# nilsfriess/dune-ddm

Hardware: AMD Instinct MI355X
Metric: preconditioned CG iterations/sec (two-level additive Schwarz), 3D Poisson 10M DoF (higher is better)
Workload: dtype f64

## Files before the change

### dune-ddm_amd/__init__.py

```python
from __future__ import annotations

import ctypes
import os

import numpy as np

_HERE = os.path.dirname(os.path.abspath(__file__))
LIB_PATH = os.path.join(_HERE, "libddm_hip.so")

GENEO_AVAILABLE = True

DDM_OK, DDM_EINVAL, DDM_EHIP, DDM_ENOTIMPL, DDM_ENUMERIC, DDM_ECOMM = 0, -1, -2, -3, -4, -5


class DdmError(RuntimeError):
    def __init__(self, code, msg):
        super().__init__(f"ddm_hip error {code}: {msg}")
        self.code = code


class SolveResult(ctypes.Structure):
    _fields_ = [("iterations", ctypes.c_int32), ("converged", ctypes.c_int32), ("def0", ctypes.c_double),
                ("reduction", ctypes.c_double), ("elapsed_s", ctypes.c_double)]

# ... 104 lines not shown
    "ddm_geneo_params_default": (_I32, [ctypes.POINTER(GeneoParams)]),
    "ddm_geneo_basis": (_I32, [_P, _P, _P, _I64, _P, _P, _P, ctypes.POINTER(GeneoParams), _I64, _P, _P, _P, ctypes.POINTER(GeneoInfo)]),
    "ddm_msgfem_basis": (_I32, [_P, _P, _P, _I64, _P, _P, _P, _P, ctypes.POINTER(GeneoParams), _I64, _P, _P, _P, ctypes.POINTER(GeneoInfo)]),
    "ddm_svd_basis": (_I32, [_P, _P, _I64, _P, _P, _P, _P, _I32, _I32, _D, _I32, _P, _P, ctypes.POINTER(GeneoInfo)]),
    "ddm_harmonic_create": (_I32, [_P, _P, _I64, _P, _I64, _P, _I64, _P, _PP]),
    "ddm_harmonic_destroy": (None, [_P]),
    "ddm_harmonic_extend": (_I32, [_P, _P, _I32, _P, _I64]),
    "ddm_blockvec_gram": (_I32, [_P, _I64, _P, _P, _I64, _I32, _P, _I64, _I32, _P]),
    "ddm_blockvec_gram2_sym": (_I32, [_P, _I64, _P, _P, _I64, _P, _P, _I64, _I32, _P, _P]),
    "ddm_blockvec_rotate": (_I32, [_P, _I64, _P, _P, _I64, _I32, _P, _I32, _P, _I64, _P, _I64]),
    "ddm_dense_sym_eig_host": (_I32, [_I32, _P, _P]),
    "ddm_dense_rayleigh_ritz_host": (_I32, [_I32, _P, _P, _I32, _D, _P, _P]),
    "ddm_combined_create": (_I32, [_P, _I32, _P, _P, _P, _PP]),
    "ddm_combined_destroy": (None, [_P]),
    "ddm_combined_apply": (_I32, [_P, _P, _P, _P]),
    "ddm_cg_solve": (_I32, [_P, _P, _P, _P, _P, _D, _I32, _I32, _P, ctypes.POINTER(SolveResult)]),
    "ddm_gmres_solve": (_I32, [_P, _P, _P, _P, _P, _D, _I32, _I32, _P, ctypes.POINTER(SolveResult)]),
    "ddm_bicgstab_solve": (_I32, [_P, _P, _P, _P, _P, _D, _I32, _P, ctypes.POINTER(ctypes.c_int32), ctypes.POINTER(SolveResult)]),
    "ddm_op_apply_multi": (_I32, [_P, _P, _I32, _P, _P]),
    "ddm_op_applyscaleadd_multi": (_I32, [_P, _P, _I32, _D, _P, _P]),
    "ddm_dot_multi": (_I32, [_P, _P, _I32, _P, _P, _P]),
    "ddm_schwarz_apply_multi": (_I32, [_P, _P, _I32, _P, _P]),
    "ddm_galerkin_apply_multi": (_I32, [_P, _P, _I32, _P, _P]),
    "ddm_combined_apply_multi": (_I32, [_P, _P, _I32, _P, _P]),
    "ddm_cg_solve_multi": (_I32, [_P, _P, _P, _I32, _P, _P, _D, _I32, _P, ctypes.POINTER(SolveResult)]),
    "ddm_cg_solve_queue": (_I32, [_P, _P, _P, _I64, _I32, _P, _P, _D, _I32, _P, ctypes.POINTER(SolveResult)]),
    "ddm_bicgstab_solve_queue": (_I32, [_P, _P, _P, _I64, _I32, _P, _P, _D, _I32, _P, ctypes.POINTER(ctypes.c_int32), ctypes.POINTER(SolveResult)]),
    "ddm_gmres_solve_multi": (_I32, [_P, _P, _P, _I32, _P, _P, _D, _I32, _I32, _P, ctypes.POINTER(SolveResult)]),
    "ddm_fgmres_solve": (_I32, [_P, _P, _P, _P, _P, _D, _I32, _I32, _P, ctypes.POINTER(SolveResult)]),
    "ddm_fgmres_solve_multi": (_I32, [_P, _P, _P, _I32, _P, _P, _D, _I32, _I32, _P, ctypes.POINTER(SolveResult)]),
# ... 474 lines not shown
    MODES = {"additive": 0, "multiplicative": 1}

    def __init__(self, ctx: Context, mode="additive", op=None, schwarz=None, galerkin=None):
        if mode not in self.MODES:
            raise NotImplementedError("Unknown apply mode in CombinedPreconditioner, use either additive or multiplicative")
        self.ctx = ctx
        h = ctypes.c_void_p()
        ctx.check(ctx.lib.ddm_combined_create(ctx.h, self.MODES[mode], op.h if op else None, schwarz.h if schwarz else None,
                                              galerkin.h if galerkin else None, ctypes.byref(h)))
        self.h = h
        self._keep = (op, schwarz, galerkin)

    def apply(self, x, d):
        self.ctx.check(self.ctx.lib.ddm_combined_apply(self.ctx.h, self.h, _ptr(x), _ptr(d)))

    def apply_multi(self, X, D):
        self.ctx.check(self.ctx.lib.ddm_combined_apply_multi(self.ctx.h, self.h, _ncols(X, D), _ptr(X), _ptr(D)))

    def check_status(self):
        self.ctx.check(self.ctx.lib.ddm_combined_status(self.ctx.h, self.h))


def cg_solve(ctx: Context, op: NonOverlappingOperator, prec: CombinedPreconditioner, x, b, reduction=1e-10, maxit=1000,
             fixed_iterations=0, history=True):
    res = SolveResult()
    hist = np.zeros(max(maxit, fixed_iterations) + 1, dtype=np.float64) if history else None
    ctx.check(ctx.lib.ddm_cg_solve(ctx.h, op.h, prec.h, _ptr(x), _ptr(b), float(reduction), int(maxit), int(fixed_iterations),
                                   _hp(hist), ctypes.byref(res)))
    return res, (hist[:res.iterations + 1] if history else None)

# ... 297 lines not shown
def dia_windows_host(A):
    lib = load_library()
    n = A.shape[0]
    rp, ci, va = _np(A.indptr, np.int64), _np(A.indices, np.int32), _np(A.data, np.float64)
    max_segs, max_runs = n + 1, 32 * (n + 1)
    segs = np.zeros((max_segs, 4), dtype=np.int32)
    runs = np.zeros((max_runs, 3), dtype=np.int32)
    counts = np.zeros(4, dtype=np.int64)
    rc = lib.ddm_dia_windows_host(n, _hp(rp), _hp(ci), _hp(va), max_segs, _hp(segs), max_runs, _hp(runs), _hp(counts))
    if rc != DDM_OK:
        raise ValueError("ddm_dia_windows_host: bad arguments")
    out = [dict(staged=bool(s[0]), window=int(s[2]), runs=[tuple(r) for r in runs[s[3]:s[3] + s[1]].tolist()]) for s in segs[:counts[0]]]
    return out, int(counts[2])


def blockvec_gram(ctx: Context, sub_ptr, U, V):
    bp = _np(sub_ptr, np.int64)
    assert U.is_contiguous() and V.is_contiguous() and U.shape[0] == V.shape[0] == bp[-1]
    out = np.empty((len(bp) - 1, U.shape[1], V.shape[1]), dtype=np.float64)
    ctx.check(ctx.lib.ddm_blockvec_gram(ctx.h, len(bp) - 1, _hp(bp), _ptr(U), U.stride(0), U.shape[1], _ptr(V), V.stride(0), V.shape[1], _hp(out)))
    return out


def blockvec_gram2_sym(ctx: Context, sub_ptr, U, V1, V2):
    bp = _np(sub_ptr, np.int64)
    p = U.shape[1]
    assert V1.shape == U.shape == V2.shape and V1.stride(0) == V2.stride(0) and U.shape[0] == bp[-1]
    g1 = np.empty((len(bp) - 1, p, p), dtype=np.float64)
    g2 = np.empty_like(g1)
    ctx.check(ctx.lib.ddm_blockvec_gram2_sym(ctx.h, len(bp) - 1, _hp(bp), _ptr(U), U.stride(0), _ptr(V1), _ptr(V2), V1.stride(0), p, _hp(g1), _hp(g2)))
# ... 9 lines not shown
```

### dune-ddm_amd/csrc/ddm_hip.hip

```cpp
#include "../../include/ddm_hip.h"

#include <dlfcn.h>
#include <rccl/rccl.h>

#include <algorithm>
#include <atomic>
#include <chrono>
#include <cmath>
#include <cstdarg>
#include <cstdio>
#include <cstdlib>
#include <cstring>
#include <deque>
#include <map>
#include <memory>
#include <mutex>
#include <string>
#include <thread>
#include <type_traits>
#include <vector>

#include "host_vec.hpp"
#include "device_buffer.hpp"
#include "kernels.hpp"
// ... 8 lines not shown

using namespace ddm;

#include "context.hpp"
#include "csr.hpp"
#include "local_factor.hpp"
#include "tri_levels.hpp"
#include "tri_csr.hpp"
#include "engine_xcd2.hpp"
#include "engine_pipe.hpp"
#include "engine_box.hpp"
#include "local_solve.hpp"
#include "local_solver.hpp"
#include "geneo.hpp"
#include "halo.hpp"
#include "preconditioners.hpp"
#include "krylov.hpp"

extern "C" int ddm_dense_sym_eig_host(int n, double *V, double *w) { return dense::sym_eig(n, V, w) ? DDM_OK : DDM_ENUMERIC; }
extern "C" int ddm_dense_rayleigh_ritz_host(int p, const double *gA, const double *gC, int keep, double tau, double *mu, double *Y)
{
  return dense::rayleigh_ritz(p, gA, gC, keep, tau, mu, Y);
}
extern "C" int ddm_dense_sym_pinv_host(int m, const double *W, double tol, double *Wpinv, int *rank)
{
  if (m < 1 || !W || !Wpinv || !rank || W == Wpinv || !(tol > 0.0 && tol < 1.0)) return fail(nullptr, DDM_EINVAL, "ddm_dense_sym_pinv_host: bad arguments");
  return dense::sym_pinv(m, W, tol, Wpinv, rank) ? DDM_OK : DDM_ENUMERIC;
}
extern "C" int ddm_dense_bgmres_factor_host(int p, const double *G, const double *scale2, double tol, double *S, double *C, int *rank)
{
// ... 22 lines not shown
```

### dune-ddm_amd/csrc/halo.hpp

```cpp
#pragma once

struct ddm_halo {
  int tag = 0, mode = 0;
  int64_t nsend = 0, nrecv = 0, ndst = 0, self_off_send = 0, self_off_recv = 0, self_count = 0;
  dbuf<int64_t> send_idx, dst_idx, dst_ptr, src_pos;
  dbuf<double> sendbuf, recvbuf;
  bool remote = false;
  std::vector<int64_t> send_counts, recv_counts;
  dbuf<double> msend, mrecv;
  int mcols = 0;
};

extern "C" int ddm_halo_create(ddm_ctx *ctx, int tag, int mode, int64_t nsend, const int64_t *send_idx,
                               const int64_t *send_counts, const int64_t *recv_counts, int64_t ndst, const int64_t *dst_idx,
                               const int64_t *dst_ptr, const int64_t *src_pos, ddm_halo **out)
{
  if (!ctx || !out || (mode != 0 && mode != 1)) return fail(ctx, DDM_EINVAL, "ddm_halo_create: bad arguments");
  auto H = std::make_unique<ddm_halo>();
  H->tag = tag;
  H->mode = mode;
  H->nsend = nsend;
  H->ndst = ndst;
  H->send_counts.assign(send_counts, send_counts + ctx->nranks);
  H->recv_counts.assign(recv_counts, recv_counts + ctx->nranks);
// ... 2 lines not shown
    if (r == ctx->rank) {
      H->self_off_send = ssum;
      H->self_off_recv = rsum;
      H->self_count = send_counts[r];
      if (send_counts[r] != recv_counts[r]) return fail(ctx, DDM_EINVAL, "halo: self send/recv counts differ");
    } else if (send_counts[r] || recv_counts[r])
      H->remote = true;
    ssum += send_counts[r];
    rsum += recv_counts[r];
  }
  if (ssum != nsend) return fail(ctx, DDM_EINVAL, "halo: send_counts do not sum to nsend");
  H->nrecv = rsum;
  const int64_t nsrc = ndst > 0 ? dst_ptr[ndst] : 0;
  for (int64_t k = 0; k < nsrc; ++k)
    if (src_pos[k] < 0 || src_pos[k] >= rsum) return fail(ctx, DDM_EINVAL, "halo: src_pos out of range");
  int rc = upload(ctx, send_idx, nsend, H->send_idx);
  if (!rc) rc = upload(ctx, dst_idx, ndst, H->dst_idx);
  if (!rc) rc = upload(ctx, dst_ptr, ndst + 1, H->dst_ptr);
  if (!rc) rc = upload(ctx, src_pos, nsrc, H->src_pos);
  if (!rc && H->sendbuf.alloc(nsend) != hipSuccess) rc = DDM_EHIP;
  if (!rc && H->recvbuf.alloc(rsum) != hipSuccess) rc = DDM_EHIP;
  if (rc) return fail(ctx, rc, "halo: device allocation failed");
  *out = H.release();
  return DDM_OK;
}
extern "C" void ddm_halo_destroy(ddm_halo *H) { delete H; }
extern "C" double *ddm_halo_sendbuf(ddm_halo *H) { return H->sendbuf; }
extern "C" double *ddm_halo_recvbuf(ddm_halo *H) { return H->recvbuf; }

static int halo_wire_rccl(ddm_ctx *ctx, const ddm_halo *H, int64_t m, const double *send, double *recv)
// ... 81 lines not shown
```

### dune-ddm_amd/csrc/kernels.hpp

```cpp
#pragma once
#include <hip/hip_runtime.h>
#include <stdint.h>

namespace ddm {

constexpr int WG = 256;
constexpr int SPMV_NNZ = 2048;
constexpr int RED_MAX_BLOCKS = 1024;
constexpr int RED_TRIPS = 4;

__device__ __forceinline__ int xcd_remap(int orig, int nwg)
{
  const int q = nwg >> 3, r = nwg & 7, xcd = orig & 7;
  return (xcd < r ? xcd * (q + 1) : r * (q + 1) + (xcd - r) * q) + (orig >> 3);
}

__device__ __forceinline__ double wave_sum(double v)
{
#pragma unroll
  for (int o = 32; o > 0; o >>= 1) v += __shfl_down(v, o, 64);
  return v;
}

__device__ __forceinline__ double block_sum(double v, double *lds4)
// ... 1074 lines not shown
      if (own[u]) s += a[u] * b[u];
  }
  for (; i < n; i += step)
    if (!MASKED || mask[i]) s += x[i] * y[i];
  s = block_sum(s, red);
  if (threadIdx.x == 0) partial[blockIdx.x] = s;
}
__global__ __launch_bounds__(WG) void k_reduce_final(int nb, const double *__restrict__ partial, double *__restrict__ out)
{
  __shared__ double red[4];
  double s = 0.0;
  for (int i = threadIdx.x; i < nb; i += WG) s += partial[i];
  s = block_sum(s, red);
  if (threadIdx.x == 0) out[0] = s;
}

__global__ void k_cg_lambda(double *scal) { scal[2] = scal[0] / scal[1]; }
__global__ void k_cg_beta(double *scal)
{
  scal[4] = scal[3] / scal[0];
  scal[0] = scal[3];
}
__global__ void k_cg_update(int64_t n, const double *__restrict__ scal, const double *__restrict__ p,
                            const double *__restrict__ q, double *__restrict__ x, double *__restrict__ b)
{
  const double lam = scal[2];
  for (int64_t i = blockIdx.x * (int64_t)WG + threadIdx.x; i < n; i += (int64_t)gridDim.x * WG) {
    x[i] += lam * p[i];
    b[i] -= lam * q[i];
  }
// ... 321 lines not shown
```

### dune-ddm_amd/csrc/krylov.hpp

```cpp
#pragma once

struct StreamDrain {
  ddm_ctx *ctx;
  ~StreamDrain() { (void)hipStreamSynchronize(ctx->stream); }
};

static void solve_result_reset(ddm_solve_result *res) { *res = ddm_solve_result{0, 0, 0.0, 1.0, 0.0}; }
enum class Defect0 { NaN, Zero, Go };
static Defect0 classify_initial_defect(double def0) { return !(def0 == def0) ? Defect0::NaN : def0 < 1e-30 ? Defect0::Zero : Defect0::Go; }
static int krylov_finish(ddm_ctx *ctx, const ddm_combined *prec, int rc, std::chrono::steady_clock::time_point t0, double *elapsed_s)
{
  (void)hipStreamSynchronize(ctx->stream);
  *elapsed_s = std::chrono::duration<double>(std::chrono::steady_clock::now() - t0).count();
  if (rc || !prec->schwarz) return rc;
  int st = 0;
  rc = ddm_ilu0_status(ctx, prec->schwarz->solver, &st);
  if (!rc && st) rc = fail(ctx, DDM_ENUMERIC, "persistent triangular solve timed out waiting for a level (results invalid)");
  return rc;
}

struct MultiFrame {
  ddm_ctx *ctx;
  const char *what;
  int m;
// ... 82 lines not shown
extern "C" void ddm_cg_end(ddm_ctx *ctx, ddm_cg *S)
{
  if (ctx) ctx->piggy = nullptr;
  if (!S) return;
  if (ctx) (void)hipStreamSynchronize(ctx->stream);
  delete S;
}
extern "C" double ddm_cg_def0(const ddm_cg *S) { return S->def0; }
extern "C" int ddm_cg_steps(ddm_ctx *ctx, ddm_cg *S, int k)
{
  struct PiggyGuard { ddm_ctx *ctx; ~PiggyGuard() { ctx->piggy = nullptr; } } piggy_guard{ctx};
  double *scal = ctx->scal;
  const int G = grid_for(S->n);
  for (int i = 0; i < k; ++i) {
    const bool first = S->it == 0;
    DDMCHECK(ddm_combined_apply(ctx, S->prec, first ? S->p : S->q, S->b));
    DDMCHECK(dot_device(ctx, S->n, S->op->owner, first ? S->p : S->q, S->b, scal + (first ? 0 : 3)));
    if (!first) {
      hipLaunchKernelGGL(k_cg_beta, dim3(1), dim3(1), 0, ctx->stream, scal);
      hipLaunchKernelGGL(k_cg_direction, dim3(G), dim3(WG), 0, ctx->stream, S->n, scal, S->q, S->p);
    }
    DDMCHECK(ddm_op_apply(ctx, S->op, S->p, S->q));
    DDMCHECK(dot_device(ctx, S->n, S->op->owner, S->p, S->q, scal + 1));
    hipLaunchKernelGGL(k_cg_lambda, dim3(1), dim3(1), 0, ctx->stream, scal);
    {
      const int nb = grid_for(S->n, WG * 4, RED_MAX_BLOCKS);
      if (S->op->owner)
        hipLaunchKernelGGL(k_cg_update_norm<true>, dim3(nb), dim3(WG), 0, ctx->stream, S->n, scal, S->op->owner, S->p, S->q, S->x, S->b, ctx->partial);
      else
        hipLaunchKernelGGL(k_cg_update_norm<false>, dim3(nb), dim3(WG), 0, ctx->stream, S->n, scal, S->op->owner, S->p, S->q, S->x, S->b, ctx->partial);
      hipLaunchKernelGGL(k_reduce_final, dim3(1), dim3(WG), 0, ctx->stream, nb, ctx->partial, scal + 5);
      if (i + 1 < k && S->prec->galerkin) ctx->piggy = scal + 5;
// ... 1559 lines not shown
```

### dune-ddm_amd/csrc/preconditioners.hpp

```cpp
#pragma once

static int dot_device(ddm_ctx *ctx, int64_t n, const uint8_t *mask, const double *x, const double *y, double *result_dev)
{
  const int nb = grid_for(n, WG * 4, RED_MAX_BLOCKS);
  if (mask)
    hipLaunchKernelGGL(k_dot_partial<true>, dim3(nb), dim3(WG), 0, ctx->stream, n, mask, x, y, ctx->partial);
  else
    hipLaunchKernelGGL(k_dot_partial<false>, dim3(nb), dim3(WG), 0, ctx->stream, n, mask, x, y, ctx->partial);
  hipLaunchKernelGGL(k_reduce_final, dim3(1), dim3(WG), 0, ctx->stream, nb, ctx->partial, result_dev);
  HIPCHECK(ctx, hipGetLastError());
  DDMCHECK(ctx_allreduce(ctx, result_dev, 1, "scalar product"));
  return DDM_OK;
}

template <class Launch>
static void for_column_groups(int m, Launch &&launch)
{
  for (int c0 = 0; c0 < m;) {
    const int cb = m - c0 >= 8 ? 8 : m - c0 >= 4 ? 4 : m - c0 >= 2 ? 2 : 1;
    launch(c0, cb);
    c0 += cb;
  }
}
#define DDM_MULTI_CB_DISPATCH(KERNEL, MASKED, cb, ...)                                                                 \
  do {                                                                                                                 \
    if (MASKED) {                                                                                                      \
      if (cb == 8) hipLaunchKernelGGL((KERNEL<8, true>), __VA_ARGS__);                                                 \
// ... 136 lines not shown
  DDMCHECK(dot_multi_device(ctx, op->n, op->owner, nrhs, X, Y, out));
  return ddm_memcpy_d2h(ctx, result_host, out, sizeof(double) * (size_t)nrhs);
}

struct ddm_schwarz {
  int64_t n = 0, n_novlp = 0;
  int type = 1;
  ddm_ilu0 *solver = nullptr;
  dbuf<int32_t> ext_map;
  dbuf<double> pou;
  dbuf<double> d_ovlp, x_ovlp;
  ddm_halo *copy = nullptr, *add = nullptr;
  dbuf<double> md_ovlp, mx_ovlp;
  int mcols = 0;
  bool multi_f32 = false;
  ~ddm_schwarz() { ddm_ilu0_destroy(solver); }
};
extern "C" int ddm_schwarz_create(ddm_ctx *ctx, const ddm_csr *A_dir, int64_t nblocks, const int64_t *block_ptr, int64_t n_novlp,
                                  const int32_t *ext_map_host, const double *pou_host, int type, ddm_halo *ovlp_copy,
                                  ddm_halo *ovlp_add, ddm_schwarz **out)
{
  return ddm_schwarz_create_ex(ctx, A_dir, nblocks, block_ptr, n_novlp, ext_map_host, pou_host, type, "ilu0", ovlp_copy, ovlp_add, out);
}
extern "C" int ddm_schwarz_create_ex(ddm_ctx *ctx, const ddm_csr *A_dir, int64_t nblocks, const int64_t *block_ptr, int64_t n_novlp,
                                     const int32_t *ext_map_host, const double *pou_host, int type, const char *subdomain_solver,
                                     ddm_halo *ovlp_copy, ddm_halo *ovlp_add, ddm_schwarz **out)
{
  if (!ctx || !A_dir || !out || !ext_map_host) return fail(ctx, DDM_EINVAL, "ddm_schwarz_create: bad arguments");
  const std::string st = subdomain_solver ? subdomain_solver : "ilu0";
  const bool direct = st == "cholmod" || st == "direct" || st == "cholesky" || st == "umfpack" || st == "ldl";
// ... 38 lines not shown
extern "C" int ddm_schwarz_engine(const ddm_schwarz *S) { return S ? ddm_ilu0_engine(S->solver) : -1; }
extern "C" ddm_ilu0 *ddm_schwarz_local_solver(ddm_schwarz *S) { return S ? S->solver : nullptr; }
extern "C" int ddm_schwarz_status(ddm_ctx *ctx, const ddm_schwarz *S)
{
  if (!S) return fail(ctx, DDM_EINVAL, "ddm_schwarz_status: bad arguments");
  int st = 0;
  DDMCHECK(ddm_ilu0_status(ctx, S->solver, &st));
  if (st) return fail(ctx, DDM_ENUMERIC, "local triangular solve timed out waiting for a dependency (code %d): results are invalid", st);
  return DDM_OK;
}
static int local_status_check(ddm_ctx *ctx, const ddm_schwarz *S)
{
  if (const unsigned e = S ? ilu0_peek_status(S->solver) : 0u)
    return fail(ctx, DDM_ENUMERIC, "an earlier local triangular solve timed out waiting for a dependency (code %u): results since then are invalid", e);
  return DDM_OK;
}
static int schwarz_apply_impl(ddm_ctx *ctx, ddm_schwarz *S, double *x, const double *d, bool acc)
{
  DDMCHECK(local_status_check(ctx, S));
  {
    ScopedTimer t(ctx, "Schwarz/get defect");
    hipLaunchKernelGGL(k_extend, dim3(grid_for(S->n)), dim3(WG), 0, ctx->stream, S->n, S->ext_map, d, S->d_ovlp);
    DDMCHECK(ddm_halo_exchange(ctx, S->copy, S->d_ovlp));
  }
  {
    ScopedTimer t(ctx, "Schwarz/local solve");
    DDMCHECK(ddm_ilu0_solve(ctx, S->solver, S->d_ovlp, S->x_ovlp));
  }
  {
    ScopedTimer t(ctx, "Schwarz/add solution");
// ... 255 lines not shown
      hipLaunchKernelGGL(k_coarse_restrict_partial, dim3(nchunk), dim3(WG), 0, ctx->stream, (int)nleft, n, left, y, chunks, partial, nchunk);
    hipLaunchKernelGGL(k_coarse_restrict_final, dim3(1), dim3(WG), 0, ctx->stream, 1, (int)nleft, d_scp, partial, d_cidx, nleft, outd + j * nleft);
  }
  if (!rc) rc = ddm_memcpy_d2h(ctx, out_host, outd, sizeof(double) * (size_t)(nleft * nright));
  return rc;
}

constexpr bool OVERLAP_DEFAULT = true;
constexpr int OVERLAP_WAVES_PER_16_CU = 7, OVERLAP_KMAX_MEASURED = 20;
static int overlap_default_grid(int num_cu, int64_t kmax)
{
  const int64_t k = std::max<int64_t>(kmax, OVERLAP_KMAX_MEASURED);
  const int64_t g = (OVERLAP_WAVES_PER_16_CU * num_cu * k + 16 * OVERLAP_KMAX_MEASURED - 1) / (16 * OVERLAP_KMAX_MEASURED);
  return (int)std::max<int64_t>(1, std::min<int64_t>(g, num_cu));
}
struct ddm_combined {
  int mode = 0;
  ddm_op *op = nullptr;
  ddm_schwarz *schwarz = nullptr;
  ddm_galerkin *galerkin = nullptr;
  dbuf<double> dnext;
  int64_t n = 0;
  bool fused = false;
  int overlap = 0;
  int side_grid = 0;
  dbuf<double> mdnext, mp, mq;
  dbuf<double> mxw, mbw;
  dbuf<int64_t> mqueue_tab;
  dbuf<double> mrt, mv, my;
  dbuf<double> mz;
  int mcols = 0, mcg_cols = 0, mqueue_cols = 0, mbicg_cols = 0, mbcg_cols = 0;
};
extern "C" int ddm_combined_create(ddm_ctx *ctx, int mode, ddm_op *op, ddm_schwarz *schwarz, ddm_galerkin *galerkin, ddm_combined **out)
{
  if (!ctx || !out || !schwarz) return fail(ctx, DDM_EINVAL, "ERROR: No preconditioners added yet");
  if (mode != 0 && mode != 1) return fail(ctx, DDM_ENOTIMPL, "Unknown apply mode in CombinedPreconditioner, use either additive or multiplicative");
  if (mode == 1 && galerkin && !op) return fail(ctx, DDM_EINVAL, "ERROR: ApplyMode is multiplicative but operator A is not provided. Set with `set_op`");
  auto C = std::make_unique<ddm_combined>();
  C->mode = mode;
  C->op = op;
  C->schwarz = schwarz;
  C->galerkin = galerkin;
  C->n = schwarz->n_novlp;
  if (mode == 0 && galerkin) {
    const char *f = std::getenv("DDM_FUSE_LEVELS");
    const char *e = std::getenv("DDM_OVERLAP_COARSE");
    const char *g = std::getenv("DDM_OVERLAP_GRID");
    C->fused = !(f && f[0] == '0') && galerkin->copy == schwarz->copy && galerkin->add == schwarz->add && galerkin->n == schwarz->n && galerkin->n_novlp == schwarz->n_novlp;
    if (C->fused && (ctx->nranks == 1 || ctx->rccl)) C->overlap = e ? (e[0] == '1' ? 1 : 0) : (OVERLAP_DEFAULT ? 2 : 0);
    C->side_grid = g ? std::max(1, std::atoi(g)) : overlap_default_grid(ctx->num_cu, galerkin->kmax);
  }
  if (C->dnext.alloc(C->n) != hipSuccess) return fail(ctx, DDM_EHIP, "combined: allocation failed");
  *out = C.release();
  return DDM_OK;
}
extern "C" int ddm_combined_status(ddm_ctx *ctx, const ddm_combined *C)
{
  if (!C) return fail(ctx, DDM_EINVAL, "ddm_combined_status: bad arguments");
  return C->schwarz ? ddm_schwarz_status(ctx, C->schwarz) : DDM_OK;
}
extern "C" void ddm_combined_destroy(ddm_combined *C) { delete C; }
static int combined_apply_fused(ddm_ctx *ctx, ddm_combined *C, double *x, const double *d)
{
  ddm_schwarz *S = C->schwarz;
  ddm_galerkin *G = C->galerkin;
  bool pipe_engine = false;
  if (C->overlap != 0) DDMCHECK(ilu0_is_pipe(ctx, S->solver, &pipe_engine));
  const bool two_streams = C->overlap == 1 || (C->overlap == 2 && pipe_engine);
  if (two_streams) DDMCHECK(ctx_side_stream(ctx));
  {
    ScopedTimer t(ctx, "Schwarz/get defect");
    hipLaunchKernelGGL(k_extend, dim3(grid_for(S->n)), dim3(WG), 0, ctx->stream, S->n, S->ext_map, d, S->d_ovlp);
    DDMCHECK(ddm_halo_exchange(ctx, S->copy, S->d_ovlp));
  }
  auto timed_chain = [&](int spread_grid) -> int {
    ScopedTimer t(ctx, "GalerkinPrec/apply");
    return coarse_chain(ctx, G, S->d_ovlp, spread_grid);
  };
  if (two_streams) {
    HIPCHECK(ctx, hipEventRecord(ctx->ev_fork, ctx->stream));
    hipStream_t main = ctx->stream;
    HIPCHECK(ctx, hipStreamWaitEvent(ctx->side, ctx->ev_fork, 0));
    ctx->stream = ctx->side;
    const int rc = timed_chain(C->side_grid);
    const hipError_t e = hipEventRecord(ctx->ev_join, ctx->side);
    ctx->stream = main;
    if (rc) return rc;
    if (e != hipSuccess) return fail(ctx, DDM_EHIP, "hipEventRecord failed: %s", hipGetErrorString(e));
// ... 1 lines not shown
  const double *pou = S->type == 1 ? S->pou : nullptr;
  if (!two_streams) DDMCHECK(timed_chain(0));
  const bool fold = !two_streams || pipe_engine;
  {
    ScopedTimer t(ctx, "Schwarz/local solve");
    DDMCHECK(ilu0_solve_epilogue(ctx, S->solver, S->d_ovlp, S->x_ovlp, fold ? pou : nullptr, fold ? (const double *)G->x_ovlp : nullptr,
                                 two_streams && fold ? ctx->ev_join : nullptr));
  }
  {
    ScopedTimer t(ctx, "Schwarz/add solution");
    if (!fold) {
      if (pou) hipLaunchKernelGGL(k_scale, dim3(grid_for(S->n)), dim3(WG), 0, ctx->stream, S->n, pou, S->x_ovlp);
      HIPCHECK(ctx, hipStreamWaitEvent(ctx->stream, ctx->ev_join, 0));
      hipLaunchKernelGGL(k_axpy, dim3(grid_for(S->n)), dim3(WG), 0, ctx->stream, S->n, 1.0, (const double *)G->x_ovlp, S->x_ovlp);
    }
    DDMCHECK(ddm_halo_exchange(ctx, S->add, S->x_ovlp));
    hipLaunchKernelGGL((k_restrict<false, false>), dim3(grid_for(S->n)), dim3(WG), 0, ctx->stream, S->n, S->ext_map, S->x_ovlp, (const double *)nullptr, x);
    HIPCHECK(ctx, hipGetLastError());
  }
  return DDM_OK;
}

extern "C" int ddm_combined_apply(ddm_ctx *ctx, ddm_combined *C, double *x, const double *d)
{
  ScopedTimer t(ctx, "CombinedPreconditioner/apply");
  DDMCHECK(local_status_check(ctx, C->schwarz));
  if (C->mode == 0 && C->galerkin && C->fused) return combined_apply_fused(ctx, C, x, d);
  DDMCHECK(schwarz_apply_impl(ctx, C->schwarz, x, d, false));
  if (!C->galerkin) return DDM_OK;
  if (C->mode == 0) {
    static const bool no_share = std::getenv("DDM_NO_SHARED_DEFECT") != nullptr;
    const bool share = !no_share && C->galerkin->copy == C->schwarz->copy && C->galerkin->n == C->schwarz->n && C->galerkin->n_novlp == C->schwarz->n_novlp;
    return galerkin_apply_impl(ctx, C->galerkin, x, d, true, share ? C->schwarz->d_ovlp : nullptr);
  }
  HIPCHECK(ctx, hipMemcpyAsync(C->dnext, d, sizeof(double) * (size_t)C->n, hipMemcpyDeviceToDevice, ctx->stream));
  DDMCHECK(ddm_op_applyscaleadd(ctx, C->op, -1.0, x, C->dnext));
  return galerkin_apply_impl(ctx, C->galerkin, x, C->dnext, true);
}
static int combined_apply_multi_impl(ddm_ctx *ctx, ddm_combined *C, int m, double *X, const double *D)
{
  ScopedTimer t(ctx, "CombinedPreconditioner/apply");
  ddm_schwarz *S = C->schwarz;
  ddm_galerkin *G = C->galerkin;
  DDMCHECK(local_status_check(ctx, S));
  if (C->mode == 0 && G && C->fused) {
    DDMCHECK(schwarz_multi_scratch(ctx, S, m));
    DDMCHECK(galerkin_multi_scratch(ctx, G, m));
    {
      ScopedTimer t2(ctx, "Schwarz/get defect");
      hipLaunchKernelGGL(k_extend_multi, dim3(grid_for(S->n * m)), dim3(WG), 0, ctx->stream, S->n, m, S->ext_map, D, S->md_ovlp);
      DDMCHECK(halo_exchange_multi(ctx, S->copy, m, S->md_ovlp));
    }
// ... 33 lines not shown
```

### include/ddm_hip.h

```cpp
#ifndef DDM_HIP_H
#define DDM_HIP_H

#include <stdint.h>

#ifdef __cplusplus
extern "C" {
#endif

#define DDM_OK 0
#define DDM_EINVAL (-1)
#define DDM_EHIP (-2)
#define DDM_ENOTIMPL (-3)
#define DDM_ENUMERIC (-4)
#define DDM_ECOMM (-5)

typedef struct ddm_ctx ddm_ctx;
typedef struct ddm_csr ddm_csr;
typedef struct ddm_ilu0 ddm_ilu0;
typedef struct ddm_halo ddm_halo;
typedef struct ddm_op ddm_op;
typedef struct ddm_schwarz ddm_schwarz;
typedef struct ddm_galerkin ddm_galerkin;
typedef struct ddm_combined ddm_combined;

// ... 150 lines not shown
int ddm_harmonic_extend(ddm_ctx *ctx, ddm_harmonic *H, int nrhs, double *X, int64_t ldx);
int ddm_blockvec_gram(ddm_ctx *ctx, int64_t nsub, const int64_t *sub_ptr, const double *U, int64_t ldu, int pu, const double *V, int64_t ldv,
                      int pv, double *G_host);
int ddm_blockvec_gram2_sym(ddm_ctx *ctx, int64_t nsub, const int64_t *sub_ptr, const double *U, int64_t ldu, const double *V1, const double *V2, int64_t ldv, int p,
                           double *G1_host, double *G2_host);
int ddm_blockvec_rotate(ddm_ctx *ctx, int64_t nsub, const int64_t *sub_ptr, const double *U, int64_t ldu, int p, const double *Y_host, int q,
                        const double *Base, int64_t ldb, double *Out, int64_t ldo);
int ddm_dense_sym_eig_host(int n, double *V, double *w);
int ddm_dense_rayleigh_ritz_host(int p, const double *gA, const double *gC, int keep, double tau, double *mu, double *Y);

int ddm_combined_create(ddm_ctx *ctx, int mode, ddm_op *op, ddm_schwarz *schwarz, ddm_galerkin *galerkin,
                        ddm_combined **out);
void ddm_combined_destroy(ddm_combined *C);
int ddm_combined_status(ddm_ctx *ctx, const ddm_combined *C);
int ddm_combined_apply(ddm_ctx *ctx, ddm_combined *C, double *x, const double *d);

typedef struct {
  int32_t iterations;
  int32_t converged;
  double def0;
  double reduction;
  double elapsed_s;
} ddm_solve_result;
int ddm_cg_solve(ddm_ctx *ctx, ddm_op *op, ddm_combined *prec, double *x, double *b, double reduction, int maxit,
                 int fixed_iterations, double *hist_host, ddm_solve_result *res);

int ddm_gmres_solve(ddm_ctx *ctx, ddm_op *op, ddm_combined *prec, double *x, double *b, double reduction, int maxit,
                    int restart, double *hist_host, ddm_solve_result *res);

int ddm_fgmres_solve(ddm_ctx *ctx, ddm_op *op, ddm_combined *prec, double *x, double *b, double reduction, int maxit, int restart,
// ... 70 lines not shown
```

Measured before the change: 228.3.

## Precompute rank-local halo plans and fuse restriction with preconditioned dot

On a single rank the copy and add halo exchanges are turned into precomputed gather plans. The extend kernel reads directly from the right source index, so the copy exchange pass disappears. The add exchange becomes a small sum kernel over shared rows, followed by a restriction that takes owned values or the sums. That restriction also accumulates the CG dot product, which removes a separate dot kernel and extra vector reads each iteration. In exchange it adds plan-building and host-copy setup, more code paths, and depends on the halo being rank-local.

```diff
diff --git a/dune-ddm_amd/__init__.py b/dune-ddm_amd/__init__.py
--- a/dune-ddm_amd/__init__.py
+++ b/dune-ddm_amd/__init__.py
@@ -142,6 +142,9 @@
     "ddm_combined_create": (_I32, [_P, _I32, _P, _P, _P, _PP]),
     "ddm_combined_destroy": (None, [_P]),
     "ddm_combined_apply": (_I32, [_P, _P, _P, _P]),
+    "ddm_combined_apply_dot": (_I32, [_P, _P, _P, _P, ctypes.POINTER(ctypes.c_double)]),
+    "ddm_combined_local_passes": (_I32, [_P]),
+    "ddm_local_passes_host": (_I32, [_I64, _I64, _P, _I64, _I64, _P, _I64, _I64, _P, _P, _P, _P, _P, _P]),
     "ddm_cg_solve": (_I32, [_P, _P, _P, _P, _P, _D, _I32, _I32, _P, ctypes.POINTER(SolveResult)]),
     "ddm_gmres_solve": (_I32, [_P, _P, _P, _P, _P, _D, _I32, _I32, _P, ctypes.POINTER(SolveResult)]),
     "ddm_bicgstab_solve": (_I32, [_P, _P, _P, _P, _P, _D, _I32, _P, ctypes.POINTER(ctypes.c_int32), ctypes.POINTER(SolveResult)]),
@@ -646,6 +649,14 @@
     def apply(self, x, d):
         self.ctx.check(self.ctx.lib.ddm_combined_apply(self.ctx.h, self.h, _ptr(x), _ptr(d)))
 
+    def apply_dot(self, x, d):
+        r = ctypes.c_double()
+        self.ctx.check(self.ctx.lib.ddm_combined_apply_dot(self.ctx.h, self.h, _ptr(x), _ptr(d), ctypes.byref(r)))
+        return r.value
+
+    def local_passes(self):
+        return int(self.ctx.lib.ddm_combined_local_passes(self.h))
+
     def apply_multi(self, X, D):
         self.ctx.check(self.ctx.lib.ddm_combined_apply_multi(self.ctx.h, self.h, _ncols(X, D), _ptr(X), _ptr(D)))
 
@@ -973,6 +984,25 @@
     return out, int(counts[2])
 
 
+def local_passes_host(n_novlp, ext_map, copy_plan, add_plan, d, x_ovlp):
+    lib = load_library()
+    em = _np(ext_map, np.int32)
+    n = len(em)
+    d, xo = _np(d, np.float64), _np(x_ovlp, np.float64)
+    assert len(d) == n_novlp and len(xo) == n
+    args, keep = [], []
+    for plan in (copy_plan, add_plan):
+        a = [_np(plan[k], np.int64) for k in ("send_idx", "dst_idx", "dst_ptr", "src_pos")]
+        keep.append(a)
+        args += [len(a[0]), len(a[1]), (ctypes.c_void_p * 4)(*[x.ctypes.data for x in a])]
+    d_ovlp, z = np.full(n, np.nan), np.full(n_novlp, np.nan)
+    counts = np.zeros(3, dtype=np.int64)
+    rc = lib.ddm_local_passes_host(n, int(n_novlp), _hp(em), *args, _hp(d), _hp(d_ovlp), _hp(xo), _hp(z), _hp(counts))
+    if rc != DDM_OK:
+        raise ValueError("ddm_local_passes_host: bad arguments")
+    return (d_ovlp, z, dict(sums=int(counts[1]), sources=int(counts[2]))) if counts[0] else None
+
+
 def blockvec_gram(ctx: Context, sub_ptr, U, V):
     bp = _np(sub_ptr, np.int64)
     assert U.is_contiguous() and V.is_contiguous() and U.shape[0] == V.shape[0] == bp[-1]
diff --git a/dune-ddm_amd/csrc/ddm_hip.hip b/dune-ddm_amd/csrc/ddm_hip.hip
--- a/dune-ddm_amd/csrc/ddm_hip.hip
+++ b/dune-ddm_amd/csrc/ddm_hip.hip
@@ -46,6 +46,7 @@
 #include "local_solver.hpp"
 #include "geneo.hpp"
 #include "halo.hpp"
+#include "local_passes.hpp"
 #include "preconditioners.hpp"
 #include "krylov.hpp"
 
diff --git a/dune-ddm_amd/csrc/halo.hpp b/dune-ddm_amd/csrc/halo.hpp
--- a/dune-ddm_amd/csrc/halo.hpp
+++ b/dune-ddm_amd/csrc/halo.hpp
@@ -4,6 +4,7 @@
   int tag = 0, mode = 0;
   int64_t nsend = 0, nrecv = 0, ndst = 0, self_off_send = 0, self_off_recv = 0, self_count = 0;
   dbuf<int64_t> send_idx, dst_idx, dst_ptr, src_pos;
+  std::vector<int64_t> h_send_idx, h_dst_idx, h_dst_ptr, h_src_pos;
   dbuf<double> sendbuf, recvbuf;
   bool remote = false;
   std::vector<int64_t> send_counts, recv_counts;
@@ -40,6 +41,10 @@
   const int64_t nsrc = ndst > 0 ? dst_ptr[ndst] : 0;
   for (int64_t k = 0; k < nsrc; ++k)
     if (src_pos[k] < 0 || src_pos[k] >= rsum) return fail(ctx, DDM_EINVAL, "halo: src_pos out of range");
+  H->h_send_idx.assign(send_idx, send_idx + nsend);
+  H->h_dst_idx.assign(dst_idx, dst_idx + ndst);
+  H->h_dst_ptr.assign(dst_ptr, dst_ptr + ndst + 1);
+  H->h_src_pos.assign(src_pos, src_pos + nsrc);
   int rc = upload(ctx, send_idx, nsend, H->send_idx);
   if (!rc) rc = upload(ctx, dst_idx, ndst, H->dst_idx);
   if (!rc) rc = upload(ctx, dst_ptr, ndst + 1, H->dst_ptr);
diff --git a/dune-ddm_amd/csrc/kernels.hpp b/dune-ddm_amd/csrc/kernels.hpp
--- a/dune-ddm_amd/csrc/kernels.hpp
+++ b/dune-ddm_amd/csrc/kernels.hpp
@@ -1112,6 +1112,62 @@
   s = block_sum(s, red);
   if (threadIdx.x == 0) out[0] = s;
 }
+__global__ void k_extend_local(int64_t n, const int32_t *__restrict__ gsrc, const double *__restrict__ d, double *__restrict__ dov)
+{
+  for (int64_t i = blockIdx.x * (int64_t)WG + threadIdx.x; i < n; i += (int64_t)gridDim.x * WG) {
+    const int32_t g = gsrc[i];
+    dov[i] = g >= 0 ? d[g] : 0.0;
+  }
+}
+__global__ void k_halo_sum_local(int64_t nsum, const int32_t *__restrict__ row, const int32_t *__restrict__ ptr, const int32_t *__restrict__ src,
+                                 const double *__restrict__ xov, double *__restrict__ sums)
+{
+  for (int64_t t = blockIdx.x * (int64_t)WG + threadIdx.x; t < nsum; t += (int64_t)gridDim.x * WG) {
+    double s = xov[row[t]];
+    for (int32_t k = ptr[t]; k < ptr[t + 1]; ++k) s = s + xov[src[k]];
+    sums[t] = s;
+  }
+}
+__device__ __forceinline__ double local_row_value(int32_t r, const double *__restrict__ xov, const double *__restrict__ sums)
+{
+  return r >= 0 ? xov[r] : sums[-(r + 1)];
+}
+template <bool DOT, bool MASKED>
+__global__ __launch_bounds__(WG) void k_restrict_local(int64_t n, const int32_t *__restrict__ own_row, const double *__restrict__ xov,
+                                                        const double *__restrict__ sums, const uint8_t *__restrict__ mask,
+                                                        const double *__restrict__ y, double *__restrict__ z, double *__restrict__ partial)
+{
+  __shared__ double red[4];
+  double s = 0.0;
+  const int64_t step = (int64_t)gridDim.x * WG;
+  int64_t i = blockIdx.x * (int64_t)WG + threadIdx.x;
+  for (; i + (RED_TRIPS - 1) * step < n; i += RED_TRIPS * step) {
+    int32_t r[RED_TRIPS];
+    double a[RED_TRIPS], b[RED_TRIPS];
+    bool own[RED_TRIPS];
+#pragma unroll
+    for (int u = 0; u < RED_TRIPS; ++u) r[u] = own_row[i + u * step];
+#pragma unroll
+    for (int u = 0; u < RED_TRIPS; ++u) {
+      a[u] = local_row_value(r[u], xov, sums);
+      b[u] = DOT ? y[i + u * step] : 0.0;
+      own[u] = DOT && (!MASKED || mask[i + u * step]);
+    }
+#pragma unroll
+    for (int u = 0; u < RED_TRIPS; ++u) {
+      z[i + u * step] = a[u];
+      if (own[u]) s += a[u] * b[u];
+    }
+  }
+  for (; i < n; i += step) {
+    const double a = local_row_value(own_row[i], xov, sums);
+    z[i] = a;
+    if (DOT && (!MASKED || mask[i])) s += a * y[i];
+  }
+  if (!DOT) return;
+  s = block_sum(s, red);
+  if (threadIdx.x == 0) partial[blockIdx.x] = s;
+}
 
 __global__ void k_cg_lambda(double *scal) { scal[2] = scal[0] / scal[1]; }
 __global__ void k_cg_beta(double *scal)
diff --git a/dune-ddm_amd/csrc/krylov.hpp b/dune-ddm_amd/csrc/krylov.hpp
--- a/dune-ddm_amd/csrc/krylov.hpp
+++ b/dune-ddm_amd/csrc/krylov.hpp
@@ -120,8 +120,7 @@
   const int G = grid_for(S->n);
   for (int i = 0; i < k; ++i) {
     const bool first = S->it == 0;
-    DDMCHECK(ddm_combined_apply(ctx, S->prec, first ? S->p : S->q, S->b));
-    DDMCHECK(dot_device(ctx, S->n, S->op->owner, first ? S->p : S->q, S->b, scal + (first ? 0 : 3)));
+    DDMCHECK(combined_apply_dot(ctx, S->prec, S->op->owner, first ? S->p : S->q, S->b, scal + (first ? 0 : 3)));
     if (!first) {
       hipLaunchKernelGGL(k_cg_beta, dim3(1), dim3(1), 0, ctx->stream, scal);
       hipLaunchKernelGGL(k_cg_direction, dim3(G), dim3(WG), 0, ctx->stream, S->n, scal, S->q, S->p);
diff --git a/dune-ddm_amd/csrc/local_passes.hpp b/dune-ddm_amd/csrc/local_passes.hpp
--- /dev/null
+++ b/dune-ddm_amd/csrc/local_passes.hpp
@@ -0,0 +1,117 @@
+#pragma once
+
+struct LocalPlan {
+  std::vector<int32_t> gsrc;
+  std::vector<int32_t> sum_row, sum_ptr, sum_src;
+  std::vector<int32_t> own_row;
+};
+struct HaloIndex {
+  int64_t nsend = 0, ndst = 0;
+  const int64_t *send_idx = nullptr, *dst_idx = nullptr, *dst_ptr = nullptr, *src_pos = nullptr;
+};
+static bool local_plan_halo_ok(const HaloIndex &H, int64_t n, std::vector<uint8_t> &seen)
+{
+  if (H.nsend < 0 || H.ndst < 0) return false;
+  for (int64_t k = 0; k < H.nsend; ++k)
+    if (H.send_idx[k] < 0 || H.send_idx[k] >= n) return false;
+  if (H.ndst == 0) return true;
+  if (H.dst_ptr[0] < 0) return false;
+  seen.assign((size_t)n, 0);
+  for (int64_t t = 0; t < H.ndst; ++t) {
+    const int64_t i = H.dst_idx[t];
+    if (i < 0 || i >= n || seen[(size_t)i] || H.dst_ptr[t + 1] < H.dst_ptr[t]) return false;
+    seen[(size_t)i] = 1;
+  }
+  if (H.dst_ptr[H.ndst] >= INT32_MAX) return false;
+  for (int64_t k = H.dst_ptr[0]; k < H.dst_ptr[H.ndst]; ++k)
+    if (H.src_pos[k] < 0 || H.src_pos[k] >= H.nsend) return false;
+  return true;
+}
+static bool local_plan_build(int64_t n, int64_t n_novlp, const int32_t *ext_map, const HaloIndex &copy, const HaloIndex &add, LocalPlan &P)
+{
+  if (n < 0 || n_novlp < 0 || n >= INT32_MAX || n_novlp >= INT32_MAX) return false;
+  for (int64_t i = 0; i < n; ++i)
+    if (ext_map[i] >= n_novlp) return false;
+  std::vector<uint8_t> seen;
+  if (!local_plan_halo_ok(copy, n, seen) || !local_plan_halo_ok(add, n, seen)) return false;
+  P.gsrc.assign(ext_map, ext_map + n);
+  for (int64_t t = 0; t < copy.ndst; ++t) {
+    const int64_t b = copy.dst_ptr[t], e = copy.dst_ptr[t + 1];
+    P.gsrc[(size_t)copy.dst_idx[t]] = e > b ? ext_map[copy.send_idx[copy.src_pos[e - 1]]] : -1;
+  }
+  P.own_row.assign((size_t)n_novlp, INT32_MIN);
+  for (int64_t i = 0; i < n; ++i) {
+    const int32_t m = ext_map[i];
+    if (m < 0) continue;
+    if (P.own_row[(size_t)m] != INT32_MIN) return false;
+    P.own_row[(size_t)m] = (int32_t)i;
+  }
+  for (int32_t r : P.own_row)
+    if (r == INT32_MIN) return false;
+  P.sum_row.clear(), P.sum_src.clear();
+  P.sum_ptr.assign(1, 0);
+  for (int64_t t = 0; t < add.ndst; ++t) {
+    const int64_t i = add.dst_idx[t];
+    const int32_t m = ext_map[i];
+    if (m < 0) continue;
+    P.own_row[(size_t)m] = -(int32_t)(P.sum_row.size() + 1);
+    P.sum_row.push_back((int32_t)i);
+    for (int64_t k = add.dst_ptr[t]; k < add.dst_ptr[t + 1]; ++k) P.sum_src.push_back((int32_t)add.send_idx[add.src_pos[k]]);
+    P.sum_ptr.push_back((int32_t)P.sum_src.size());
+  }
+  return true;
+}
+static void local_extend_host(const LocalPlan &P, const double *d, double *d_ovlp)
+{
+  for (size_t i = 0; i < P.gsrc.size(); ++i) d_ovlp[i] = P.gsrc[i] >= 0 ? d[P.gsrc[i]] : 0.0;
+}
+static void local_sum_restrict_host(const LocalPlan &P, const double *x_ovlp, double *z)
+{
+  std::vector<double> sums(P.sum_row.size());
+  for (size_t t = 0; t < P.sum_row.size(); ++t) {
+    double s = x_ovlp[P.sum_row[t]];
+    for (int32_t k = P.sum_ptr[t]; k < P.sum_ptr[t + 1]; ++k) s = s + x_ovlp[P.sum_src[(size_t)k]];
+    sums[t] = s;
+  }
+  for (size_t m = 0; m < P.own_row.size(); ++m) z[m] = P.own_row[m] >= 0 ? x_ovlp[P.own_row[m]] : sums[(size_t)(-(P.own_row[m] + 1))];
+}
+extern "C" int ddm_local_passes_host(int64_t n, int64_t n_novlp, const int32_t *ext_map, int64_t copy_nsend, int64_t copy_ndst, const int64_t *const *copy,
+                                     int64_t add_nsend, int64_t add_ndst, const int64_t *const *add, const double *d, double *d_ovlp, const double *x_ovlp,
+                                     double *z, int64_t *counts_out)
+{
+  if (n < 0 || n_novlp < 0 || !copy || !add || !counts_out || (n > 0 && (!ext_map || !d_ovlp || !x_ovlp)) || (n_novlp > 0 && (!d || !z))) return DDM_EINVAL;
+  const HaloIndex hc{copy_nsend, copy_ndst, copy[0], copy[1], copy[2], copy[3]}, ha{add_nsend, add_ndst, add[0], add[1], add[2], add[3]};
+  for (const HaloIndex *H : {&hc, &ha})
+    if ((H->nsend > 0 && !H->send_idx) || (H->ndst > 0 && (!H->dst_idx || !H->dst_ptr || (H->dst_ptr[H->ndst] > 0 && !H->src_pos)))) return DDM_EINVAL;
+  LocalPlan P;
+  const bool built = local_plan_build(n, n_novlp, ext_map, hc, ha, P);
+  counts_out[0] = built, counts_out[1] = built ? (int64_t)P.sum_row.size() : 0, counts_out[2] = built ? (int64_t)P.sum_src.size() : 0;
+  if (!built) return DDM_OK;
+  local_extend_host(P, d, d_ovlp);
+  local_sum_restrict_host(P, x_ovlp, z);
+  return DDM_OK;
+}
+
+struct LocalPlanDev {
+  dbuf<int32_t> gsrc, sum_row, sum_ptr, sum_src, own_row;
+  dbuf<double> sums;
+  int64_t nsum = 0;
+};
+static HaloIndex halo_host_index(const ddm_halo *H) { return HaloIndex{H->nsend, H->ndst, H->h_send_idx.data(), H->h_dst_idx.data(), H->h_dst_ptr.data(), H->h_src_pos.data()}; }
+static bool halo_is_rank_local(const ddm_ctx *ctx, const ddm_halo *H) { return H && ctx->nranks == 1 && !ctx->rccl_self && !H->remote && H->nrecv == H->nsend; }
+static int local_plan_upload(ddm_ctx *ctx, int64_t n, int64_t n_novlp, const int32_t *ext_map_host, const ddm_halo *copy, const ddm_halo *add,
+                             std::unique_ptr<LocalPlanDev> &out)
+{
+  LocalPlan P;
+  if (!local_plan_build(n, n_novlp, ext_map_host, halo_host_index(copy), halo_host_index(add), P)) return DDM_OK;
+  auto D = std::make_unique<LocalPlanDev>();
+  D->nsum = (int64_t)P.sum_row.size();
+  DDMCHECK(upload(ctx, P.gsrc.data(), n, D->gsrc));
+  DDMCHECK(upload(ctx, P.sum_row.data(), D->nsum, D->sum_row));
+  DDMCHECK(upload(ctx, P.sum_ptr.data(), D->nsum + 1, D->sum_ptr));
+  DDMCHECK(upload(ctx, P.sum_src.data(), (int64_t)P.sum_src.size(), D->sum_src));
+  DDMCHECK(upload(ctx, P.own_row.data(), n_novlp, D->own_row));
+  HIPCHECK(ctx, D->sums.alloc(D->nsum));
+  out = std::move(D);
+  return DDM_OK;
+}
diff --git a/dune-ddm_amd/csrc/preconditioners.hpp b/dune-ddm_amd/csrc/preconditioners.hpp
--- a/dune-ddm_amd/csrc/preconditioners.hpp
+++ b/dune-ddm_amd/csrc/preconditioners.hpp
@@ -1,5 +1,12 @@
 #pragma once
 
+static int dot_finish(ddm_ctx *ctx, int64_t n, double *result_dev)
+{
+  const int nb = grid_for(n, WG * 4, RED_MAX_BLOCKS);
+  hipLaunchKernelGGL(k_reduce_final, dim3(1), dim3(WG), 0, ctx->stream, nb, ctx->partial, result_dev);
+  HIPCHECK(ctx, hipGetLastError());
+  return ctx_allreduce(ctx, result_dev, 1, "scalar product");
+}
 static int dot_device(ddm_ctx *ctx, int64_t n, const uint8_t *mask, const double *x, const double *y, double *result_dev)
 {
   const int nb = grid_for(n, WG * 4, RED_MAX_BLOCKS);
@@ -7,10 +14,7 @@
     hipLaunchKernelGGL(k_dot_partial<true>, dim3(nb), dim3(WG), 0, ctx->stream, n, mask, x, y, ctx->partial);
   else
     hipLaunchKernelGGL(k_dot_partial<false>, dim3(nb), dim3(WG), 0, ctx->stream, n, mask, x, y, ctx->partial);
-  hipLaunchKernelGGL(k_reduce_final, dim3(1), dim3(WG), 0, ctx->stream, nb, ctx->partial, result_dev);
-  HIPCHECK(ctx, hipGetLastError());
-  DDMCHECK(ctx_allreduce(ctx, result_dev, 1, "scalar product"));
-  return DDM_OK;
+  return dot_finish(ctx, n, result_dev);
 }
 
 template <class Launch>
@@ -177,6 +181,8 @@
   dbuf<double> md_ovlp, mx_ovlp;
   int mcols = 0;
   bool multi_f32 = false;
+  std::unique_ptr<LocalPlanDev> local;
+  bool local_tried = false;
   ~ddm_schwarz() { ddm_ilu0_destroy(solver); }
 };
 extern "C" int ddm_schwarz_create(ddm_ctx *ctx, const ddm_csr *A_dir, int64_t nblocks, const int64_t *block_ptr, int64_t n_novlp,
@@ -245,6 +251,15 @@
   if (const unsigned e = S ? ilu0_peek_status(S->solver) : 0u)
     return fail(ctx, DDM_ENUMERIC, "an earlier local triangular solve timed out waiting for a dependency (code %u): results since then are invalid", e);
   return DDM_OK;
+}
+static int schwarz_local_plan(ddm_ctx *ctx, ddm_schwarz *S)
+{
+  if (S->local_tried) return DDM_OK;
+  S->local_tried = true;
+  if (!halo_is_rank_local(ctx, S->copy) || !halo_is_rank_local(ctx, S->add)) return DDM_OK;
+  std::vector<int32_t> ext_map((size_t)S->n);
+  if (S->n > 0) DDMCHECK(ddm_memcpy_d2h(ctx, ext_map.data(), S->ext_map, (int64_t)sizeof(int32_t) * S->n));
+  return local_plan_upload(ctx, S->n, S->n_novlp, ext_map.data(), S->copy, S->add, S->local);
 }
 static int schwarz_apply_impl(ddm_ctx *ctx, ddm_schwarz *S, double *x, const double *d, bool acc)
 {
@@ -530,6 +545,7 @@
   const int64_t g = (OVERLAP_WAVES_PER_16_CU * num_cu * k + 16 * OVERLAP_KMAX_MEASURED - 1) / (16 * OVERLAP_KMAX_MEASURED);
   return (int)std::max<int64_t>(1, std::min<int64_t>(g, num_cu));
 }
+enum { LOCAL_EXTEND = 2, LOCAL_SUM = 4, LOCAL_ALL = LOCAL_EXTEND | LOCAL_SUM };
 struct ddm_combined {
   int mode = 0;
   ddm_op *op = nullptr;
@@ -540,6 +556,7 @@
   bool fused = false;
   int overlap = 0;
   int side_grid = 0;
+  int local = 0;
   dbuf<double> mdnext, mp, mq;
   dbuf<double> mxw, mbw;
   dbuf<int64_t> mqueue_tab;
@@ -566,6 +583,12 @@
     if (C->fused && (ctx->nranks == 1 || ctx->rccl)) C->overlap = e ? (e[0] == '1' ? 1 : 0) : (OVERLAP_DEFAULT ? 2 : 0);
     C->side_grid = g ? std::max(1, std::atoi(g)) : overlap_default_grid(ctx->num_cu, galerkin->kmax);
   }
+  if (C->fused) {
+    const char *l = std::getenv("DDM_LOCAL_PASSES");
+    const int v = l ? std::atoi(l) : 1, want = v == 1 ? LOCAL_ALL : v & LOCAL_ALL;
+    if (want) DDMCHECK(schwarz_local_plan(ctx, schwarz));
+    if (schwarz->local) C->local = want;
+  }
   if (C->dnext.alloc(C->n) != hipSuccess) return fail(ctx, DDM_EHIP, "combined: allocation failed");
   *out = C.release();
   return DDM_OK;
@@ -576,18 +599,27 @@
   return C->schwarz ? ddm_schwarz_status(ctx, C->schwarz) : DDM_OK;
 }
 extern "C" void ddm_combined_destroy(ddm_combined *C) { delete C; }
-static int combined_apply_fused(ddm_ctx *ctx, ddm_combined *C, double *x, const double *d)
+extern "C" int ddm_combined_local_passes(const ddm_combined *C) { return C ? C->local : 0; }
+static int combined_apply_fused(ddm_ctx *ctx, ddm_combined *C, double *x, const double *d, bool dot = false, const uint8_t *mask = nullptr)
 {
   ddm_schwarz *S = C->schwarz;
   ddm_galerkin *G = C->galerkin;
+  const LocalPlanDev *L = S->local.get();
+  const auto count_exchange = [&](const ddm_halo *H) { ctx->n_halo_groups += H->nsend != 0 || H->ndst != 0; };
+  if (dot && !(C->local & LOCAL_SUM)) return fail(ctx, DDM_EINVAL, "combined_apply_fused: the dot product needs the rank-local sum pass");
   bool pipe_engine = false;
   if (C->overlap != 0) DDMCHECK(ilu0_is_pipe(ctx, S->solver, &pipe_engine));
   const bool two_streams = C->overlap == 1 || (C->overlap == 2 && pipe_engine);
   if (two_streams) DDMCHECK(ctx_side_stream(ctx));
   {
     ScopedTimer t(ctx, "Schwarz/get defect");
-    hipLaunchKernelGGL(k_extend, dim3(grid_for(S->n)), dim3(WG), 0, ctx->stream, S->n, S->ext_map, d, S->d_ovlp);
-    DDMCHECK(ddm_halo_exchange(ctx, S->copy, S->d_ovlp));
+    if (C->local & LOCAL_EXTEND) {
+      hipLaunchKernelGGL(k_extend_local, dim3(grid_for(S->n)), dim3(WG), 0, ctx->stream, S->n, (const int32_t *)L->gsrc, d, S->d_ovlp);
+      count_exchange(S->copy);
+    } else {
+      hipLaunchKernelGGL(k_extend, dim3(grid_for(S->n)), dim3(WG), 0, ctx->stream, S->n, S->ext_map, d, S->d_ovlp);
+      DDMCHECK(ddm_halo_exchange(ctx, S->copy, S->d_ovlp));
+    }
   }
   auto timed_chain = [&](int spread_grid) -> int {
     ScopedTimer t(ctx, "GalerkinPrec/apply");
@@ -619,8 +651,22 @@
       HIPCHECK(ctx, hipStreamWaitEvent(ctx->stream, ctx->ev_join, 0));
       hipLaunchKernelGGL(k_axpy, dim3(grid_for(S->n)), dim3(WG), 0, ctx->stream, S->n, 1.0, (const double *)G->x_ovlp, S->x_ovlp);
     }
-    DDMCHECK(ddm_halo_exchange(ctx, S->add, S->x_ovlp));
-    hipLaunchKernelGGL((k_restrict<false, false>), dim3(grid_for(S->n)), dim3(WG), 0, ctx->stream, S->n, S->ext_map, S->x_ovlp, (const double *)nullptr, x);
+    if (C->local & LOCAL_SUM) {
+      const int64_t n = S->n_novlp;
+      const dim3 nb(grid_for(n, WG * 4, RED_MAX_BLOCKS));
+      const int32_t *own_row = L->own_row;
+      const double *xov = S->x_ovlp, *sums = L->sums;
+      if (L->nsum > 0)
+        hipLaunchKernelGGL(k_halo_sum_local, dim3(grid_for(L->nsum)), dim3(WG), 0, ctx->stream, L->nsum, (const int32_t *)L->sum_row, (const int32_t *)L->sum_ptr,
+                           (const int32_t *)L->sum_src, xov, L->sums.get());
+      count_exchange(S->add);
+      if (!dot) hipLaunchKernelGGL((k_restrict_local<false, false>), nb, dim3(WG), 0, ctx->stream, n, own_row, xov, sums, mask, d, x, ctx->partial.get());
+      else if (mask) hipLaunchKernelGGL((k_restrict_local<true, true>), nb, dim3(WG), 0, ctx->stream, n, own_row, xov, sums, mask, d, x, ctx->partial.get());
+      else hipLaunchKernelGGL((k_restrict_local<true, false>), nb, dim3(WG), 0, ctx->stream, n, own_row, xov, sums, mask, d, x, ctx->partial.get());
+    } else {
+      DDMCHECK(ddm_halo_exchange(ctx, S->add, S->x_ovlp));
+      hipLaunchKernelGGL((k_restrict<false, false>), dim3(grid_for(S->n)), dim3(WG), 0, ctx->stream, S->n, S->ext_map, S->x_ovlp, (const double *)nullptr, x);
+    }
     HIPCHECK(ctx, hipGetLastError());
   }
   return DDM_OK;
@@ -641,6 +687,26 @@
   HIPCHECK(ctx, hipMemcpyAsync(C->dnext, d, sizeof(double) * (size_t)C->n, hipMemcpyDeviceToDevice, ctx->stream));
   DDMCHECK(ddm_op_applyscaleadd(ctx, C->op, -1.0, x, C->dnext));
   return galerkin_apply_impl(ctx, C->galerkin, x, C->dnext, true);
+}
+static int combined_apply_dot(ddm_ctx *ctx, ddm_combined *C, const uint8_t *mask, double *x, const double *d, double *result_dev)
+{
+  if (!(C->mode == 0 && C->galerkin && C->fused && (C->local & LOCAL_SUM))) {
+    DDMCHECK(ddm_combined_apply(ctx, C, x, d));
+    return dot_device(ctx, C->n, mask, x, d, result_dev);
+  }
+  {
+    ScopedTimer t(ctx, "CombinedPreconditioner/apply");
+    DDMCHECK(local_status_check(ctx, C->schwarz));
+    DDMCHECK(combined_apply_fused(ctx, C, x, d, true, mask));
+  }
+  return dot_finish(ctx, C->n, result_dev);
+}
+extern "C" int ddm_combined_apply_dot(ddm_ctx *ctx, ddm_combined *C, double *x, const double *d, double *result_host)
+{
+  if (!ctx || !C || !C->op || !x || !d || x == d || !result_host) return fail(ctx, DDM_EINVAL, "ddm_combined_apply_dot: bad arguments (the scalar product is the operator's: the combination needs one)");
+  if (C->op->n != C->n) return fail(ctx, DDM_EINVAL, "ddm_combined_apply_dot: operator and preconditioner differ in size");
+  DDMCHECK(combined_apply_dot(ctx, C, C->op->owner, x, d, ctx->scal + 8));
+  return ddm_memcpy_d2h(ctx, result_host, ctx->scal + 8, sizeof(double));
 }
 static int combined_apply_multi_impl(ddm_ctx *ctx, ddm_combined *C, int m, double *X, const double *D)
 {
diff --git a/include/ddm_hip.h b/include/ddm_hip.h
--- a/include/ddm_hip.h
+++ b/include/ddm_hip.h
@@ -188,6 +188,11 @@
 void ddm_combined_destroy(ddm_combined *C);
 int ddm_combined_status(ddm_ctx *ctx, const ddm_combined *C);
 int ddm_combined_apply(ddm_ctx *ctx, ddm_combined *C, double *x, const double *d);
+int ddm_combined_apply_dot(ddm_ctx *ctx, ddm_combined *C, double *x, const double *d, double *result_host);
+int ddm_combined_local_passes(const ddm_combined *C);
+int ddm_local_passes_host(int64_t n, int64_t n_novlp, const int32_t *ext_map, int64_t copy_nsend, int64_t copy_ndst, const int64_t *const *copy,
+                          int64_t add_nsend, int64_t add_ndst, const int64_t *const *add, const double *d, double *d_ovlp, const double *x_ovlp,
+                          double *z, int64_t *counts_out);
 
 typedef struct {
   int32_t iterations;
```

Result: no change. 230.6, median of 6 (+1.0%).
